# NUS-HPC-AI-Lab/Dynamic-Tuning

Hardware: AMD Instinct MI355X
Metric: images/sec DyT ViT-B/16 fine-tune step (student+teacher fwd, bwd, AdamW) @ keep~0.7 (higher is better)
Workload: dtype fp16; 1 GPU; ViT-B/16 DyT on CIFAR-100 shape, batch=128/GPU, 1xMI355X per rank, keep-ratio target 0.7 (BASELINE.json configs[1]; N>1 = configs[3] shape: global batch 128*N, DP over RCCL); per_gpu_batch=128, global_batch=128, ffn_num=64, num_classes=100, train_mode=compact, parallelism=dp1, hip_graph=False

## Files before the change

dynamic-tuning_amd/_lib.py:

```python
import ctypes
import os


_HERE = os.path.dirname(os.path.abspath(__file__))
_LIB_DIR = os.environ.get("DYT_LIB_DIR", _HERE)
LIB_PATH = os.path.join(_LIB_DIR, "libdyt_hip.so")
LIB_PATH_F16 = os.path.join(_LIB_DIR, "libdyt_hip_f16.so")

PREC_FP32, PREC_BF16 = 0, 1
PREC_FP16 = 2
PREC_FP16X3F = 4
PREC_FP16X3H = 5
PREC_FP16F8 = 6
PREC_FP16X3Q = 7
PREC_FP16X3 = 3
F_TRAINING, F_COMPLETE, F_SAVE, F_MASKED_DENSE, F_GATE_ALWAYS, F_ACCUM_GRAD, F_DEVICE_SEED, F_TOKENS_IN, F_TOKENS_OUT = 1, 2, 4, 8, 16, 32, 64, 128, 256
CREATE_WIDE_HEAD = 1
OPT_STREAM_OVERLAP, OPT_CLS_TAIL, OPT_SHARE_BLOCK0, OPT_COUNT_FLOPS_TOKENS, OPT_GRAD_SCALE_LOG2, OPT_FC2_CAT, OPT_ATTN_BWD_FUSED, OPT_F32_SPLIT16, OPT_ATTN_V2, OPT_GEMM_SPLITK, OPT_LEARNABLE_SCALE = 1, 2, 3, 4, 5, 6, 7, 8, 9, 10, 11

(P_CLS, P_POS, P_PE_W, P_PE_B, P_LN1_W, P_LN1_B, P_QKV_W, P_QKV_B, P_PROJ_W, P_PROJ_B, P_LN2_W, P_LN2_B,
 P_FC1_W, P_FC1_B, P_FC2_W, P_FC2_B, P_NORM_W, P_NORM_B, P_AD_DOWN_W, P_AD_DOWN_B, P_AD_UP_W, P_AD_UP_B,
 P_GATE_W, P_GATE_B, P_HEAD_W, P_HEAD_B,
 P_POOL_QUERY, P_POOL_NQ_W, P_POOL_NQ_B, P_POOL_NK_W, P_POOL_NK_B, P_POOL_NV_W, P_POOL_NV_B, P_POOL_Q_W, P_POOL_K_W,
 P_POOL_V_W, P_POOL_Q_BIAS, P_POOL_V_BIAS, P_POOL_PROJ_W, P_POOL_PROJ_B, P_AD_SCALE, P_AD_LN_W, P_AD_LN_B, P_COUNT) = range(44)
# ... 48 lines not shown
                ("inference_only", ctypes.c_int32)]


class DyTError(RuntimeError):
    pass


def inference_only_default(explicit=None, tuning_config=None):
    if explicit is not None:
        return bool(explicit)
    try:
        v = getattr(tuning_config, "dyt_inference_only")
    except (AttributeError, KeyError):
        v = None
    if v is not None:
        return bool(v)
    return os.environ.get("DYT_INFERENCE_ONLY", "0").strip().lower() not in ("", "0", "false", "no", "off")


def wide_head_default(explicit=None, tuning_config=None, num_classes=0):
    if explicit is not None:
        return bool(explicit)
    try:
        v = getattr(tuning_config, "dyt_wide_head")
    except (AttributeError, KeyError):
        v = None
    if v is not None:
        return bool(v)
    e = os.environ.get("DYT_WIDE_HEAD")
    if e is not None and e.strip() != "":
        return e.strip().lower() not in ("0", "false", "no", "off")
    return int(num_classes) > 1024


_lib = None

_vp, _i, _i64, _f, _u64 = ctypes.c_void_p, ctypes.c_int, ctypes.c_int64, ctypes.c_float, ctypes.c_uint64

SYMBOLS = {
    "dyt_last_error": (ctypes.c_char_p, []),
    "dyt_version": (_i, []),
    "dyt_operand_type": (_i, []),
    "dyt_ctx_create": (_i, [ctypes.POINTER(Config), ctypes.POINTER(_vp)]),
    "dyt_ctx_create_ex": (_i, [ctypes.POINTER(Config), ctypes.c_uint32, ctypes.POINTER(_vp)]),
    "dyt_ctx_destroy": (_i, [_vp]),
    "dyt_ctx_bytes": (_i, [_vp, ctypes.POINTER(_i64)]),
    "dyt_ctx_set_option": (_i, [_vp, _i, _i]),
    "dyt_set_global_option": (_i, [_i, _i]),
    "dyt_set_drop_path": (_i, [_vp, _f]),
    "dyt_set_drop_path_scales": (_i, [_vp, _i, _vp]),
    "dyt_set_soft_targets": (_i, [_vp, _vp, _i]),
    "dyt_set_frozen": (_i, [_vp, _i, _i, _vp, _vp]),
    "dyt_trainable_numel": (_i, [_vp, ctypes.POINTER(_i64)]),
    "dyt_trainable_offset": (_i, [_vp, _i, _i, ctypes.POINTER(_i64), ctypes.POINTER(_i64)]),
    "dyt_forward": (_i, [_vp, _i, _vp, _i, _i, _vp, _vp, _vp, _vp, _u64, _vp, _vp, _vp, _vp]),
    "dyt_backward": (_i, [_vp, _i, _vp, _vp, _vp, _vp, _vp, _vp]),
    "dyt_loss": (_i, [_vp, _i, _vp, _vp, _vp, _i, _f, _f, _f, _f, _vp, _vp, _vp, _vp, _vp]),
    "dyt_adamw": (_i, [_vp, _vp, _vp, _vp, _i64, _i, _f, _f, _f, _f, _f, _f, _vp]),
    "dyt_adamw_guarded": (_i, [_vp, _vp, _vp, _vp, _i64, _vp, _f, _f, _f, _f, _f, _f, _vp]),
    "dyt_step_fwd_bwd": (_i, [_vp, _vp, _vp, _i, _i, _vp, _vp, _vp, _vp, _u64, _f, _f, _f, _f, _vp, _vp, _vp, _vp,
                              _vp, _vp]),
    "dyt_seed": (_i, [_vp, _u64, _vp]),
    "dyt_grad_part": (_i, [_vp, _i, ctypes.POINTER(_i64), ctypes.POINTER(_i64)]),
    "dyt_stream_wait_grads": (_i, [_vp, _i, _vp]),
    "dyt_allreduce_grads": (_i, [_vp, _vp, _vp, _vp, _vp]),
    "dyt_clip_grad_norm": (_i, [_vp, _vp, _i64, _f, _f, _vp, _vp]),
    "dyt_debug_dispatch": (_i, [_vp, _i, _i, _vp, _vp, _vp, _vp, _vp]),
    "dyt_debug_dact": (_i, [_vp, _i, _i, _vp, _vp, _vp]),
    "dyt_debug_drop_path": (_i, [_vp, _i, _vp, _vp]),
    "dyt_layernorm": (_i, [_vp, _vp, _vp, _vp, _i, _vp]),
    "dyt_linear": (_i, [_vp, _vp, _vp, _vp, _i, _i, _i, _i, _vp]),
    "dyt_linear_split": (_i, [_vp, _vp, _vp, _vp, _i, _i, _i, _i, _vp]),
    "dyt_attention": (_i, [_vp, _vp, _vp, _vp, _i, _i, _vp]),
    "dyt_adapter_fwd": (_i, [_vp, _vp, _vp, _vp, _vp, _vp, _vp, _i, _i, _f, _f, _vp, _u64, _i, _vp]),
    "dyt_adapter_bwd": (_i, [_vp, _vp, _vp, _vp, _vp, _vp, _vp, _vp, _vp, _vp, _i, _i, _f, _f, _vp, _u64, _i, _vp]),
    "dyt_head_wide": (_i, [_vp, _vp, _vp, _vp, _vp, _vp, _vp, _vp, _vp, _vp, _i, _i, _vp]),
    "dyt_mlp_gathered_fwd": (_i, [_vp, _i, _vp, _vp, _vp, _i, _vp, _vp]),
    "dyt_mlp_gathered_bwd": (_i, [_vp, _i, _vp, _vp, _vp, _vp, _i, _vp]),
    "dyt_gate_compact": (_i, [_vp, _vp, _vp, _vp, _vp, _i, _i, _f, _f, _vp, _vp, _vp, _vp, _vp, _vp]),
    "dyt_gemm_bf16_raw": (_i, [_vp, _vp, _vp, _i, _i, _i, _i, _vp]),
    "dyt_gemm_f32_raw": (_i, [_vp, _vp, _vp, _i, _i, _i, _i, _vp]),
    "dyt_wgrad_scratch_floats": (ctypes.c_int64, [_i]),
    "dyt_wgrad_raw": (_i, [_vp, _vp, _i, _i, _i, _vp, _vp, _vp, _vp, _vp]),
    "dyt_debug_counters": (_i, [ctypes.POINTER(ctypes.c_uint64), _i]),
    "dyt_debug_checksums": (_i, [_i, ctypes.POINTER(ctypes.c_uint64), _i, ctypes.POINTER(_i)]),
    "dyt_debug_checksum_label": (ctypes.c_char_p, [_i, _i]),
    "dyt_debug_dump_read": (ctypes.c_int64, [_vp, _i64]),
    "dyt_profile_enable": (_i, [_vp, _i]),
    "dyt_profile_read": (_i, [_vp, _i, ctypes.POINTER(ctypes.c_double), ctypes.POINTER(_i64),
                              ctypes.POINTER(ctypes.c_double)]),
}


_lib16 = None


def lib(fp16=False):
    global _lib, _lib16
    if fp16:
        if _lib16 is None:
            lib()
            if not os.path.exists(LIB_PATH_F16):
                raise DyTError("%s not found: build it with `make -C dynamic-tuning_amd/csrc`" % LIB_PATH_F16)
            L = ctypes.CDLL(LIB_PATH_F16)
            for name, (res, args) in SYMBOLS.items():
                fn = getattr(L, name)
                fn.restype = res
                fn.argtypes = args
            if L.dyt_operand_type() != 1:
                raise DyTError("%s was not built with -DDYT_FP16" % LIB_PATH_F16)
            _lib16 = L
        return _lib16
    if _lib is None:
        if not os.path.exists(LIB_PATH):
            raise DyTError("%s not found: build it with `make -C dynamic-tuning_amd/csrc` "
                           "(or __graft_entry__.build()); the DyT path has no fallback" % LIB_PATH)
        import torch
        rt = os.path.join(os.path.dirname(torch.__file__), "lib", "libamdhip64.so")
        if not os.path.exists(rt):
            raise DyTError("PyTorch-ROCm's HIP runtime not found at %s" % rt)
        ctypes.CDLL(rt, mode=ctypes.RTLD_GLOBAL)
        rccl = os.path.join(os.path.dirname(torch.__file__), "lib", "librccl.so")
        if os.path.exists(rccl):
            ctypes.CDLL(rccl, mode=ctypes.RTLD_GLOBAL)
        L = ctypes.CDLL(LIB_PATH)
        for name, (res, args) in SYMBOLS.items():
            fn = getattr(L, name)
            fn.restype = res
            fn.argtypes = args
        _lib = L
    return _lib


def check(rc, L=None):
    if rc != 0:
        msg = (L or lib()).dyt_last_error().decode()
        if not msg and _lib16 is not None and L is None:
            msg = _lib16.dyt_last_error().decode()
        raise DyTError("libdyt_hip: %s (code %d)" % (msg, rc))


def ptr(t):
    if t is None:
        return None
    assert t.is_cuda and t.is_contiguous(), "libdyt_hip needs contiguous device tensors"
    return ctypes.c_void_p(t.data_ptr())


def stream_ptr():
    import torch
    return ctypes.c_void_p(torch.cuda.current_stream().cuda_stream)


class _NcclUniqueId(ctypes.Structure):
    _fields_ = [("internal", ctypes.c_byte * 128)]


_rccl = None


def rccl():
    global _rccl
    if _rccl is None:
        import torch
        path = os.path.join(os.path.dirname(torch.__file__), "lib", "librccl.so")
        if not os.path.exists(path):
# ... 62 lines not shown
```

dynamic-tuning_amd/csrc/rowops.hip:

```cpp
#include <stdlib.h>
#include <algorithm>
#include "kernels.h"
#include "rowhelp.h"

namespace dyt {

#define LAUNCH_CHECK() DYT_HIP_CHECK(hipGetLastError())

#if defined(DYT_NOPIN_LN) || defined(DYT_NOPIN_ROWS)
#define LN_ROWPIN(x)
#else
#define LN_ROWPIN(x) (x).landed()
#endif
#if defined(DYT_NOPIN_LN) || defined(DYT_NOPIN_SCALARS)
#define LN_SCALPIN3(a, b, c)
#else
#define LN_SCALPIN3(a, b, c) DYT_PIN3(a, b, c)
#endif
#if defined(DYT_NOPIN_TOK) || defined(DYT_NOPIN_ROWS)
#define TK_ROWPIN(x)
#else
#define TK_ROWPIN(x) (x).landed()
#endif
#if defined(DYT_NOPIN_TOK) || defined(DYT_NOPIN_SCALARS)
// ... 830 lines not shown
        for (int i = threadIdx.x; i < nparts; i += 64) acc += part[i];
        acc = wave_sum(acc);
        if (threadIdx.x == 0) {
            const float norm = sqrtf(acc) * fabsf(pre_scale);
            coef_s = fminf(1.0f, max_norm / (norm + 1e-6f));
            if (blockIdx.x == 0 && norm_out) norm_out[0] = norm;
        }
    }
    __syncthreads();
    const float coef = coef_s;
    if (coef >= 1.0f) return;
    for (int64_t i = (int64_t)blockIdx.x * 256 + threadIdx.x; i < n; i += (int64_t)gridDim.x * 256) g[i] *= coef;
}
int launch_clip_grad_norm(float* g, int64_t n, float max_norm, float pre_scale, float* scratch, float* norm_out, hipStream_t s) {
    const int nparts = 256;
    hipLaunchKernelGGL(sqsum_kernel, dim3(nparts), dim3(256), 0, s, g, n, scratch);
    hipLaunchKernelGGL(clip_scale_kernel, dim3(nparts), dim3(256), 0, s, g, n, scratch, nparts, max_norm, pre_scale, norm_out);
    LAUNCH_CHECK();
    return 0;
}

int launch_adamw(float* p, const float* g, float* m, float* v, int64_t n, float lr, float b1, float b2, float eps,
                 float wd, float bc1, float rsqrt_bc2, float gscale, hipStream_t s) {
    hipLaunchKernelGGL(adamw_kernel, dim3((unsigned)((n + 255) / 256)), dim3(256), 0, s, p, g, m, v, n, lr, b1, b2, eps,
                       wd, bc1, rsqrt_bc2, gscale);
    LAUNCH_CHECK();
    return 0;
}

template <class AT>
__global__ __launch_bounds__(256) void bwd_prep_kernel(const float* __restrict__ g, const AT* __restrict__ h,
                                                       const int* __restrict__ dst_of, const float* __restrict__ row_mask,
                                                       AT* __restrict__ g_at, AT* __restrict__ dH,
                                                       float* __restrict__ dmask, int M, float gs) {
    const int lane = threadIdx.x & 63;
    const int t = blockIdx.x * 4 + (threadIdx.x >> 6);
    if (t >= M) return;
    Row12 gr;
    gr.load(g + (size_t)t * D, lane);
    int r = dst_of ? dst_of[t] : t;
    float mk = row_mask ? row_mask[t] : 1.0f;
    gr.landed(); DYT_PIN2(r, mk);
    if (g_at) {
        Row12 gsc;
#pragma unroll
        for (int i = 0; i < 12; ++i) gsc.v[i] = gr.v[i] * gs;
        gsc.store(g_at + (size_t)t * D, lane);
    }
    float dm = 0.f;
    if (r >= 0) {
        if (h) {
            Row12 hr;
            hr.load_at(h + (size_t)r * D, lane);
            hr.landed();
            dm = dot12(gr, hr);
        }
        if (dH) {
            if (row_mask) {
#pragma unroll
                for (int i = 0; i < 12; ++i) gr.v[i] *= mk;
            }
#pragma unroll
            for (int i = 0; i < 12; ++i) gr.v[i] *= gs;
            gr.store(dH + (size_t)r * D, lane);
        }
    }
    if (dmask && lane == 0) dmask[t] = dm;
}
int launch_bwd_prep(int precision, const BwdPrepArgs& a, hipStream_t s) {
    const int grid = (a.M + 3) / 4;
    if (precision == 0)
        hipLaunchKernelGGL(bwd_prep_kernel<float>, dim3(grid), dim3(256), 0, s, a.g, (const float*)a.h, a.dst_of, a.row_mask,
                           (float*)a.g_at, (float*)a.dH, a.dmask, a.M, 1.0f);
    else
        hipLaunchKernelGGL(bwd_prep_kernel<bf16>, dim3(grid), dim3(256), 0, s, a.g, (const bf16*)a.h, a.dst_of, a.row_mask,
                           (bf16*)a.g_at, (bf16*)a.dH, a.dmask, a.M, a.gs);
    LAUNCH_CHECK();
    return 0;
}

constexpr int TOK_PER_BLOCK = 32;

template <class AT>
__global__ __launch_bounds__(256) void tok_bwd_kernel(TokBwdArgs a) {
    __shared__ float red[4][D + 1];
    const int tid = threadIdx.x, lane = tid & 63, wave = tid >> 6;
    Row12 wg, ln2w, dwg;
    float dbg = 0.f;
#pragma unroll
    for (int i = 0; i < 12; ++i) dwg.v[i] = 0.f;
    if (a.gate_w) { wg.load(a.gate_w, lane); TK_ROWPIN(wg); }
    if (a.dA2) { ln2w.load(a.ln2_w, lane); TK_ROWPIN(ln2w); }
    const int t0 = blockIdx.x * TOK_PER_BLOCK;
    int rv = -1;
    if (a.dA2 && a.write_du) {
        const int tt = t0 + wave + 4 * lane;
        if (lane < TOK_PER_BLOCK / 4 && tt < a.M) {
            if (a.g_cls) { const int bb = tt / NT; rv = (tt - bb * NT == 0) ? bb : -1; }
            else rv = a.dst_of ? a.dst_of[tt] : tt;
        }
    }
    for (int k = wave; k < TOK_PER_BLOCK; k += 4) {
        const int t = t0 + k;
        if (t >= a.M) break;
        const int b = t / NT, n = t - b * NT;
        Row12 du, ur, e, dy;
        const bool need_u = (a.dA2 && (!a.g_cls || n == 0)) || a.gate_w;
        const bool gate = a.gate_w && n >= 1;
        const bool cat = gate && a.cat_dact && a.dmask;
        if (need_u) ur.load_nt(a.u + (size_t)t * D, lane);
        const bool du16 = a.du_in_at && a.write_du && !a.g_cls;
        if (du16) du.load_at(reinterpret_cast<const AT*>(a.du_in_at) + (size_t)t * D, lane);
        else if (a.write_du && !a.g_cls) du.load(a.du + (size_t)t * D, lane);
        else if (a.write_du && n == 0) du.load(a.g_cls + (size_t)b * D, lane);
        else {
#pragma unroll
            for (int i = 0; i < 12; ++i) du.v[i] = 0.f;
        }
        if (a.dad) e.load_at(reinterpret_cast<const AT*>(a.dad) + (size_t)t * D, lane);
        const int r = __builtin_amdgcn_readlane(rv, k >> 2);
        if (r >= 0) dy.load_at(reinterpret_cast<const AT*>(a.dA2) + (size_t)r * D, lane);
        float2 st2 = make_float2(0.f, 1.f);
        if (a.dA2 && a.write_du) st2 = a.stats2[t];
        float ext = 0.f, sf = 0.f, dmk = 0.f, dlg = 0.f;
        float cd = 0.f, cz = 0.f;
        if (gate) {
            const size_t oi = (size_t)b * a.out_stride + n - 1;
            if (a.dtoken_select) ext = a.dtoken_select[oi];
            else if (a.dtok) ext = a.dtok[0] + (a.maskf[t] != 0.f ? a.dtok[2] : a.dtok[1]);
            sf = a.soft[t];
            if (a.dmask) dmk = a.dmask[t];
            if (a.dtoken_logits) dlg = a.dtoken_logits[oi];
            if (cat) {
                cd = to_f32(reinterpret_cast<const AT*>(a.cat_dact)[(size_t)t * RP + lane]);
                cz = to_f32(reinterpret_cast<const AT*>(a.cat_ddz)[(size_t)t * RP + lane]);
            }
        }
        if (need_u) TK_ROWPIN(ur);
        TK_ROWPIN(du);
        if (a.dad) TK_ROWPIN(e);
        if (r >= 0) TK_ROWPIN(dy);
        TK_SCALPIN3(st2.x, st2.y, ext);
        TK_SCALPIN3(sf, dmk, dlg);
        if (cat) {
            DYT_PIN2(cd, cz);
            const float czs = a.cat_ddz_dscale ? a.cat_ddz_scale * *a.cat_ddz_dscale : a.cat_ddz_scale;
            if (a.maskf[t] != 0.f) dmk -= wave_sum(cd * cz) * czs;
        }
        const float bs = a.branch_scale ? a.branch_scale[b] : 1.0f;
        dmk *= bs;
        if (du16) {
#pragma unroll
            for (int i = 0; i < 12; ++i) du.v[i] *= a.inv_gs;
        }
        if (a.dad) {
#pragma unroll
            for (int i = 0; i < 12; ++i) du.v[i] += e.v[i] * a.inv_gs;
        }
        if (a.dA2 && a.write_du) {
            if (r >= 0) {
                ln_bwd_row(dy, ur, ln2w, st2);
                const float ds = a.inv_gs * bs;
#pragma unroll
                for (int i = 0; i < 12; ++i) du.v[i] += dy.v[i] * ds;
            }
        }
        if (gate) {
            float dlogit = (dmk + ext) * sf * (1.0f - sf);
            if (a.training) dlogit /= a.tau;
            dlogit += dlg;
#pragma unroll
            for (int i = 0; i < 12; ++i) {
                du.v[i] = fmaf(dlogit, wg.v[i], du.v[i]);
                dwg.v[i] = fmaf(dlogit, ur.v[i], dwg.v[i]);
            }
            dbg += dlogit;
        }
        if (a.write_du) {
            if (a.du) du.store(a.du + (size_t)t * D, lane);
            if (a.du3) du.store_split3(reinterpret_cast<bf16*>(a.du3) + (size_t)t * SPLIT_A * D, lane, a.du3_scale, a.du3_hi_only);
            if (a.du_at) {
                Row12 dsc;
#pragma unroll
                for (int i = 0; i < 12; ++i) dsc.v[i] = du.v[i] * a.gs;
                dsc.store(reinterpret_cast<AT*>(a.du_at) + (size_t)t * D, lane);
            }
        }
    }
    if (a.gate_w) {
#pragma unroll
        for (int i = 0; i < 3; ++i)
#pragma unroll
            for (int e = 0; e < 4; ++e) red[wave][i * 256 + lane * 4 + e] = dwg.v[4 * i + e];
        if (lane == 0) red[wave][D] = dbg;
        __syncthreads();
        for (int c = tid; c < D + 1; c += 256)
            a.partial[(size_t)blockIdx.x * (D + 1) + c] = red[0][c] + red[1][c] + red[2][c] + red[3][c];
    }
}
int launch_tok_bwd(int precision, const TokBwdArgs& a, int* nblocks_out, hipStream_t s) {
    const int grid = (a.M + TOK_PER_BLOCK - 1) / TOK_PER_BLOCK;
    if (nblocks_out) *nblocks_out = grid;
    if (dbg_skip(8)) return 0;
    if (precision == 0) hipLaunchKernelGGL(tok_bwd_kernel<float>, dim3(grid), dim3(256), 0, s, a);
    else hipLaunchKernelGGL(tok_bwd_kernel<bf16>, dim3(grid), dim3(256), 0, s, a);
    LAUNCH_CHECK();
    return 0;
}

__global__ __launch_bounds__(256) void drop_path_draw_kernel(float* __restrict__ scales, int depth, int batch, float rate, uint64_t seed,
                                                             const uint64_t* __restrict__ seed_dev, uint64_t subseq_base) {
    const int i = blockIdx.x * 256 + threadIdx.x;
    if (i >= 2 * depth * batch) return;
    const int b = i % batch, l = (i / batch) % depth, branch = i / (batch * depth);
    const float drop = depth > 1 ? rate * (float)l / (float)(depth - 1) : 0.f;
    float v = 1.0f;
    if (drop > 0.f) {
        const float keep = 1.0f - drop;
        Philox ph(seed_dev ? *seed_dev : seed, subseq_base + (uint64_t)(2 * l + branch), (uint64_t)b);
        v = ph.u01(0) < keep ? 1.0f / keep : 0.0f;
    }
    scales[i] = v;
}
int launch_drop_path_draw(float* scales, int depth, int batch, float rate, uint64_t seed, const uint64_t* seed_dev, uint64_t subseq_base, hipStream_t s) {
    hipLaunchKernelGGL(drop_path_draw_kernel, dim3((2 * depth * batch + 255) / 256), dim3(256), 0, s, scales, depth, batch, rate, seed, seed_dev, subseq_base);
    LAUNCH_CHECK();
    return 0;
}
template <class AT>
__global__ __launch_bounds__(256) void scale_rows_kernel(AT* __restrict__ x, const float* __restrict__ scale, int M, int ld) {
    const size_t i = ((size_t)blockIdx.x * 256 + threadIdx.x) * 4;
    if (i >= (size_t)M * ld) return;
    const float sc = scale[(int)(i / ld) / NT];
    float v[4];
    load4(x + i, v);
    store4(x + i, v[0] * sc, v[1] * sc, v[2] * sc, v[3] * sc);
}
int launch_scale_rows(int precision, void* x, const float* scale, int M, int ld, hipStream_t s) {
    const unsigned grid = (unsigned)(((size_t)M * ld / 4 + 255) / 256);
    if (precision == 0) hipLaunchKernelGGL(scale_rows_kernel<float>, dim3(grid), dim3(256), 0, s, (float*)x, scale, M, ld);
    else hipLaunchKernelGGL(scale_rows_kernel<bf16>, dim3(grid), dim3(256), 0, s, (bf16*)x, scale, M, ld);
    LAUNCH_CHECK();
    return 0;
}

__global__ __launch_bounds__(256) void reduce_partials_kernel(const float* __restrict__ partial, int nparts, int stride,
                                                              float* __restrict__ out, int n, float alpha) {
    __shared__ float red[8][32];
    const int o = threadIdx.x & 31, grp = threadIdx.x >> 5;
    const int i = blockIdx.x * 32 + o;
    float acc = 0.f;
    if (i < n) {
        const int per = (nparts + 7) / 8;
        const int p0 = grp * per, p1 = min(nparts, p0 + per);
#pragma unroll 4
        for (int p = p0; p < p1; ++p) acc += partial[(size_t)p * stride + i];
    }
    red[grp][o] = acc;
    __syncthreads();
    if (grp == 0 && i < n) {
        float t = 0.f;
#pragma unroll
        for (int g = 0; g < 8; ++g) t += red[g][o];
        out[i] += alpha * t;
    }
}
int launch_reduce_partials(const float* partial, int nparts, int stride, float* out, int n, float alpha, hipStream_t s) {
    hipLaunchKernelGGL(reduce_partials_kernel, dim3((n + 31) / 32), dim3(256), 0, s, partial, nparts, stride, out, n, alpha);
    LAUNCH_CHECK();
    return 0;
}

struct TokReduceBatch { const float* partial[ReduceQueue::MAX_TOK]; float* out[ReduceQueue::MAX_TOK]; int nparts[ReduceQueue::MAX_TOK]; };
__global__ __launch_bounds__(256) void reduce_partials_batch_kernel(TokReduceBatch b, int stride, int n) {
    __shared__ float red[8][32];
    const float* __restrict__ partial = b.partial[blockIdx.y];
    const int nparts = b.nparts[blockIdx.y];
    const int o = threadIdx.x & 31, grp = threadIdx.x >> 5;
    const int i = blockIdx.x * 32 + o;
    float acc = 0.f;
    if (i < n) {
        const int per = (nparts + 7) / 8;
        const int p0 = grp * per, p1 = min(nparts, p0 + per);
#pragma unroll 4
        for (int p = p0; p < p1; ++p) acc += partial[(size_t)p * stride + i];
    }
    red[grp][o] = acc;
    __syncthreads();
// ... 333 lines not shown
```

dynamic-tuning_amd/csrc/unit_abi.hip:

```cpp
#include "ctx.h"

namespace dyt {

template <class AT>
__global__ void qkv_split_kernel(const float* __restrict__ qkv, AT* __restrict__ q, AT* __restrict__ k, AT* __restrict__ v,
                                 int batch) {
    const size_t idx = (size_t)blockIdx.x * 256 + threadIdx.x;
    if (idx >= (size_t)batch * NT * 3 * D) return;
    const int col = (int)(idx % (3 * D));
    const size_t row = idx / (3 * D);
    const int b = (int)(row / NT), n = (int)(row % NT);
    const int which = col / D, c = col % D, h = c >> 6, d = c & 63;
    const float val = qkv[idx] * (which == 0 ? 0.125f : 1.0f);
    AT* dst = which == 0 ? q : (which == 1 ? k : v);
    dst[(((size_t)b * NH + h) * NT + n) * HD + d] = from_f32<AT>(val);
}
template <class AT>
__global__ void to_f32_kernel(const AT* __restrict__ src, float* __restrict__ dst, size_t n) {
    const size_t i = (size_t)blockIdx.x * 256 + threadIdx.x;
    if (i < n) dst[i] = to_f32(src[i]);
}

}

extern "C" int dyt_debug_dact(dyt_ctx* c, int slot, int layer, float* out, int* rows_out, void* stream) {
    if (!c || !out || slot < 0 || slot >= c->cfg.slots || layer < 0 || layer >= c->cfg.depth) { set_error("bad slot / layer"); return DYT_ERR_ARG; }
    { int rc = refuse_inference(c, "dyt_debug_dact (per-block tensors of a saved pass)"); if (rc) return rc; }
    const Slot& S = c->slots[slot];
    if (S.batch < 1) { set_error("slot %d holds no pass", slot); return DYT_ERR_STATE; }
    hipStream_t s = static_cast<hipStream_t>(stream);
    const bool tail = c->cls_tail && layer == c->cfg.depth - 1;
    const size_t rows = tail ? (size_t)S.batch : (size_t)S.batch * NT, n = rows * RP;
    const LayerS& L = S.L[layer];
    if (rows_out) *rows_out = (int)rows;
    if (S.saved16 && L.dact16) hipLaunchKernelGGL(to_f32_kernel<bf16>, dim3((unsigned)((n + 255) / 256)), dim3(256), 0, s, (const bf16*)L.dact16, out, n);
    else if (c->prec == DYT_PREC_FP32) DYT_HIP_CHECK(hipMemcpyAsync(out, L.d_act, n * 4, hipMemcpyDeviceToDevice, s));
    else hipLaunchKernelGGL(to_f32_kernel<bf16>, dim3((unsigned)((n + 255) / 256)), dim3(256), 0, s, (const bf16*)L.d_act, out, n);
    DYT_HIP_CHECK(hipGetLastError());
    return DYT_OK;
}

extern "C" int dyt_gemm_bf16_raw(const void* a, const void* w, void* cmat, int M, int N, int K, int variant, void* stream) {
    if (!a || !w || !cmat) { set_error("null argument"); return DYT_ERR_ARG; }
    return launch_gemm_raw(a, w, cmat, M, N, K, variant, static_cast<hipStream_t>(stream));
}

extern "C" int64_t dyt_wgrad_scratch_floats(int M) { return (int64_t)((M + 511) / 512) * (D + 8) * 80; }
extern "C" int dyt_wgrad_raw(const void* X, const void* Y, int M, int r, int precision, float* partial, float* out_w, float* out_xsum,
                             float* out_ysum, void* stream) {
    if (!X || !Y || !partial || !out_w || M < 1 || r < 1 || r > RP) { set_error("bad argument"); return DYT_ERR_ARG; }
    WgradArgs a; a.X = X; a.Y = Y; a.M = M; a.r = r; a.partial = partial;
    a.out_w = out_w; a.sc = r; a.sj = 1; a.alpha = 1.0f; a.out_xsum = out_xsum; a.alpha_x = 1.0f; a.out_ysum = out_ysum; a.alpha_y = 1.0f;
    return launch_wgrad(precision, a, static_cast<hipStream_t>(stream));
}

extern "C" int dyt_gemm_f32_raw(const float* a, const float* w, float* cmat, int M, int N, int K, int variant, void* stream) {
    if (!a || !w || !cmat) { set_error("null argument"); return DYT_ERR_ARG; }
    return launch_gemm_f32_raw(a, w, cmat, M, N, K, variant, static_cast<hipStream_t>(stream));
}

extern "C" int dyt_debug_counters(uint64_t* out4, int reset) {
    if (!out4) { set_error("null argument"); return DYT_ERR_ARG; }
    return gemm_debug_counters(reinterpret_cast<unsigned long long*>(out4), reset);
}

extern "C" int dyt_layernorm(const float* x, const float* w, const float* b, float* out, int rows, void* stream) {
    if (!x || !w || !b || !out || rows < 1) { set_error("bad argument"); return DYT_ERR_ARG; }
    return launch_ln_fwd_f32out(x, w, b, out, rows, static_cast<hipStream_t>(stream));
}

struct Scratch {
    std::vector<void*> ptrs;
    ~Scratch() { for (void* p : ptrs) hipFree(p); }
    void* get(size_t bytes) {
        void* p = nullptr;
        if (hipMalloc(&p, bytes) != hipSuccess) return nullptr;
        ptrs.push_back(p);
        return p;
    }
};

extern "C" int dyt_linear(const float* a, const float* w, const float* bias, float* cmat, int M, int N, int K, int precision,
                          void* stream) {
    if (!a || !w || !cmat || M < 1) { set_error("bad argument"); return DYT_ERR_ARG; }
    hipStream_t s = static_cast<hipStream_t>(stream);
    GemmArgs g; g.M = M; g.N = N; g.K = K; g.bias = bias; g.out_f32 = cmat;
    Scratch sc;
    if (precision == 0) { g.A = a; g.W = w; }
    else {
        void* a2 = sc.get((size_t)M * K * 2); void* w2 = sc.get((size_t)N * K * 2);
        if (!a2 || !w2) { set_error("scratch alloc failed"); return DYT_ERR_HIP; }
        int rc = launch_convert(1, a, a2, (int64_t)M * K, s); if (rc) return rc;
        rc = launch_convert(1, w, w2, (int64_t)N * K, s); if (rc) return rc;
        g.A = a2; g.W = w2;
    }
    int rc = launch_gemm(precision, EPI_BIAS_F32, g, s);
    if (rc) return rc;
    DYT_HIP_CHECK(hipStreamSynchronize(s));
    return DYT_OK;
}

extern "C" int dyt_linear_split(const float* a, const float* w, const float* bias, float* cmat, int M, int N, int K, int form, void* stream) {
    if (!a || !w || !cmat || M < 1 || (form != 3 && form != 8)) { set_error("bad argument"); return DYT_ERR_ARG; }
    hipStream_t s = static_cast<hipStream_t>(stream);
    Scratch sc;
    void* a3 = sc.get((size_t)((M + 255) / 256 * 256) * SPLIT_A * K * 2); void* w3 = sc.get((size_t)N * SPLIT_A * K * 2);
    int* ew = (int*)sc.get(16); unsigned* scr = (unsigned*)sc.get(16);
    if (!a3 || !w3 || !ew || !scr) { set_error("scratch alloc failed"); return DYT_ERR_HIP; }
    int rc = form == 8 ? launch_split_w_f8(w, w3, N, K, ew, scr, s) : launch_split3_w(w, w3, N, K, s);
    if (rc) return rc;
    GemmArgs g; g.A = a; g.W = w; g.M = M; g.N = N; g.K = K; g.bias = bias; g.out_f32 = cmat; g.W3 = w3; g.a3 = a3;
    if (form == 8) { g.f8 = true; g.w_exp = ew; }
    rc = launch_gemm(0, EPI_BIAS_F32, g, s);
    if (rc) return rc;
    DYT_HIP_CHECK(hipStreamSynchronize(s));
    return DYT_OK;
}

template <class AT>
static int attention_test(const float* qkv, float* out, const float* dout, float* dqkv, int B, int P, hipStream_t s) {
    Scratch sc;
    const size_t M = (size_t)B * NT;
    AT* q = (AT*)sc.get(M * D * sizeof(AT)); AT* k = (AT*)sc.get(M * D * sizeof(AT)); AT* v = (AT*)sc.get(M * D * sizeof(AT));
    AT* o = (AT*)sc.get(M * D * sizeof(AT));
    float* lse = (float*)sc.get((size_t)B * NH * NT * 4);
    if (!q || !k || !v || !o || !lse) { set_error("scratch alloc failed"); return DYT_ERR_HIP; }
    const size_t n3 = M * 3 * D;
    hipLaunchKernelGGL(qkv_split_kernel<AT>, dim3((unsigned)((n3 + 255) / 256)), dim3(256), 0, s, qkv, q, k, v, B);
    int rc = launch_attn_fwd(P, q, k, v, o, lse, B, s);
    if (rc) return rc;
    hipLaunchKernelGGL(to_f32_kernel<AT>, dim3((unsigned)((M * D + 255) / 256)), dim3(256), 0, s, (const AT*)o, out, M * D);
    if (dout && dqkv) {
        AT* d_o = (AT*)sc.get(M * D * sizeof(AT)); AT* dq = (AT*)sc.get(n3 * sizeof(AT));
        float* delta = (float*)sc.get((size_t)B * NH * NT * 4);
        if (!d_o || !dq || !delta) { set_error("scratch alloc failed"); return DYT_ERR_HIP; }
        rc = launch_convert(P, dout, d_o, (int64_t)(M * D), s); if (rc) return rc;
// ... 302 lines not shown
```

include/dyt_hip.h:

```cpp
#ifndef DYT_HIP_H
#define DYT_HIP_H

#include <stdint.h>

#ifdef __cplusplus
extern "C" {
#endif

#define DYT_OK 0
#define DYT_ERR_ARG (-1)
#define DYT_ERR_HIP (-2)
#define DYT_ERR_STATE (-3)

#define DYT_PREC_FP32 0
#define DYT_PREC_BF16 1

#define DYT_F_TRAINING 1
#define DYT_F_COMPLETE 2
#define DYT_F_SAVE 4
#define DYT_F_MASKED_DENSE 8
#define DYT_F_ACCUM_GRAD 32
#define DYT_F_DEVICE_SEED 64
#define DYT_F_TOKENS_IN 128
#define DYT_F_TOKENS_OUT 256
// ... 70 lines not shown
int dyt_set_global_option(int option, int value);

int dyt_set_drop_path(dyt_ctx* ctx, float rate);
int dyt_set_drop_path_scales(dyt_ctx* ctx, int slot, const float* scales);

int dyt_set_frozen(dyt_ctx* ctx, int param, int layer, const float* src, void* stream);

int dyt_trainable_numel(const dyt_ctx* ctx, int64_t* numel);
int dyt_trainable_offset(const dyt_ctx* ctx, int param, int layer, int64_t* offset, int64_t* numel);

int dyt_forward(dyt_ctx* ctx, int slot, const float* images, int batch, int flags,
                const float* trainable, const float* g1, const float* g2,
                const uint8_t* keep_mask, uint64_t seed,
                float* logits, float* token_select, float* token_logits, void* stream);

int dyt_backward(dyt_ctx* ctx, int slot, const float* dlogits, const float* dtoken_select,
                 const float* dtok_uniform, const float* dtoken_logits, float* grad_flat, void* stream);

int dyt_loss(dyt_ctx* ctx, int slot_student, const float* logits_s, const float* logits_t,
             const int64_t* targets, int batch, float token_target_ratio, float token_loss_ratio,
             float token_minimal, float token_minimal_weight,
             float* dlogits_s, float* dlogits_t, float* out_losses, float* dtok, void* stream);

int dyt_set_soft_targets(dyt_ctx* ctx, const float* targets, int rows);

int dyt_adamw(float* param, const float* grad, float* exp_avg, float* exp_avg_sq, int64_t numel,
              int step, float lr, float beta1, float beta2, float eps, float weight_decay,
              float grad_scale, void* stream);

int dyt_adamw_guarded(float* param, const float* grad, float* exp_avg, float* exp_avg_sq, int64_t numel, int32_t* state,
                      float lr, float beta1, float beta2, float eps, float weight_decay, float grad_scale, void* stream);

int dyt_step_fwd_bwd(dyt_ctx* ctx, const float* images, const int64_t* targets, int batch,
                     int flags, const float* trainable,
                     const float* g1, const float* g2, const uint8_t* keep_mask, uint64_t seed,
                     float token_target_ratio, float token_loss_ratio,
                     float token_minimal, float token_minimal_weight,
                     float* grad_flat, float* out_losses, float* logits_s, float* logits_t,
                     float* token_select, void* stream);

int dyt_seed(dyt_ctx* ctx, uint64_t seed, void* stream);

int dyt_grad_part(const dyt_ctx* ctx, int part, int64_t* offset, int64_t* numel);
int dyt_stream_wait_grads(dyt_ctx* ctx, int part, void* stream);

int dyt_allreduce_grads(dyt_ctx* ctx, void* rccl_comm, float* grad_flat, void* comm_stream, void* stream);

int dyt_clip_grad_norm(dyt_ctx* ctx, float* grad, int64_t numel, float max_norm, float pre_scale, float* norm_out, void* stream);

int dyt_debug_dispatch(dyt_ctx* ctx, int slot, int layer, int32_t* row_src, int32_t* dst_of, int32_t* counts, int32_t* total,
                       void* stream);
int dyt_debug_dact(dyt_ctx* ctx, int slot, int layer, float* out, int* rows_out, void* stream);
int dyt_debug_drop_path(dyt_ctx* ctx, int slot, float* out, void* stream);

int dyt_adapter_fwd(const float* x, const float* down_w, const float* down_b, const float* up_w, const float* up_b,
                    const float* residual, float* out, int M, int r, float scale, float drop_p, const uint8_t* keep_mask,
                    uint64_t seed, int precision, void* stream);
int dyt_adapter_bwd(const float* x, const float* down_w, const float* down_b, const float* up_w, const float* dout, float* dx,
                    float* d_down_w, float* d_down_b, float* d_up_w, float* d_up_b, int M, int r, float scale, float drop_p,
                    const uint8_t* keep_mask, uint64_t seed, int precision, void* stream);
int dyt_head_wide(const float* cls_x, const float* norm_w, const float* norm_b, const float* head_w, const float* head_b,
                  float* logits, const float* dlogits, float* dx, float* d_head_w, float* d_head_b, int batch, int C, void* stream);
int dyt_mlp_gathered_fwd(dyt_ctx* ctx, int layer, const float* u, const float* mask, float* x, int batch, int32_t* total_out,
                         void* stream);
int dyt_mlp_gathered_bwd(dyt_ctx* ctx, int layer, const float* u, const float* mask, const float* dy, float* du, int batch, void* stream);

int dyt_linear_split(const float* a, const float* w, const float* bias, float* c, int M, int N, int K, int form, void* stream);

int dyt_layernorm(const float* x, const float* w, const float* b, float* out, int rows, void* stream);
int dyt_linear(const float* a, const float* w, const float* bias, float* c, int M, int N, int K,
               int precision, void* stream);
int dyt_attention(const float* qkv, float* out, const float* dout, float* dqkv, int batch,
                  int precision, void* stream);
int dyt_gate_compact(const float* u, const float* w, const float* b, const float* g1, const float* g2,
                     int batch, int training, float tau, float threshold,
                     float* mask, float* logits, int32_t* keep_idx, int32_t* counts, int32_t* total,
                     void* stream);

int dyt_gemm_bf16_raw(const void* a, const void* w, void* c, int M, int N, int K, int variant, void* stream);
int dyt_gemm_f32_raw(const float* a, const float* w, float* c, int M, int N, int K, int variant, void* stream);
int64_t dyt_wgrad_scratch_floats(int M);
int dyt_wgrad_raw(const void* X, const void* Y, int M, int r, int precision, float* partial, float* out_w, float* out_xsum,
                  float* out_ysum, void* stream);
int dyt_debug_checksums(int slot, uint64_t* out, int max_n, int* n_out);
const char* dyt_debug_checksum_label(int slot, int i);
int64_t dyt_debug_dump_read(void* dst_device, int64_t max_bytes);
int dyt_debug_counters(uint64_t* out4, int reset);
int dyt_profile_enable(dyt_ctx* ctx, int on);
int dyt_profile_read(dyt_ctx* ctx, int category, double* ms, int64_t* launches, double* flops);

#ifdef __cplusplus
}
#endif
#endif
```

Baseline: 5534 images/s.

## Specialize token-backward kernel by template and batch loads across tokens

Splits the token backward kernel into template variants keyed on gate, concat-dact and dA2 presence, so dead branches are removed at compile time. Gated variants load two tokens per wave before consuming either, to overlap memory latency. The ungated path gets a one-wave-per-token kernel. Loads half-precision rows packed rather than unpacked. Adds env-selectable schedules and a raw test entry point. The cost is more kernel instantiations and higher register pressure.

After: 5422 images/s. 2.0% lower.

```diff
diff --git a/dynamic-tuning_amd/_lib.py b/dynamic-tuning_amd/_lib.py
--- a/dynamic-tuning_amd/_lib.py
+++ b/dynamic-tuning_amd/_lib.py
@@ -154,6 +154,8 @@
     "dyt_gemm_f32_raw": (_i, [_vp, _vp, _vp, _i, _i, _i, _i, _vp]),
     "dyt_wgrad_scratch_floats": (ctypes.c_int64, [_i]),
     "dyt_wgrad_raw": (_i, [_vp, _vp, _i, _i, _i, _vp, _vp, _vp, _vp, _vp]),
+    "dyt_tok_bwd_raw": (_i, [_vp, _vp, _vp, _vp, _vp, _vp, _vp, _vp, _vp, _vp, _vp, _vp, _vp, _vp, _i, _i, _f, _vp, _vp, _i, _i, _f, _vp, _vp,
+                             _vp, _vp, _f, _vp, _vp, _vp, _f, _i, _i, ctypes.POINTER(_i), _vp]),
     "dyt_debug_counters": (_i, [ctypes.POINTER(ctypes.c_uint64), _i]),
     "dyt_debug_checksums": (_i, [_i, ctypes.POINTER(ctypes.c_uint64), _i, ctypes.POINTER(_i)]),
     "dyt_debug_checksum_label": (ctypes.c_char_p, [_i, _i]),
diff --git a/dynamic-tuning_amd/csrc/rowops.hip b/dynamic-tuning_amd/csrc/rowops.hip
--- a/dynamic-tuning_amd/csrc/rowops.hip
+++ b/dynamic-tuning_amd/csrc/rowops.hip
@@ -936,112 +936,188 @@
 constexpr int TOK_PER_BLOCK = 32;
 
 template <class AT>
-__global__ __launch_bounds__(256) void tok_bwd_kernel(TokBwdArgs a) {
-    __shared__ float red[4][D + 1];
+struct RowP {
+    typedef AT v4 __attribute__((ext_vector_type(4)));
+    v4 p[3];
+    __device__ __forceinline__ void load(const AT* q, int lane) {
+#pragma unroll
+        for (int i = 0; i < 3; ++i) p[i] = *reinterpret_cast<const v4*>(q + i * 256 + lane * 4);
+    }
+    __device__ __forceinline__ void landed() { DYT_PIN3(p[0], p[1], p[2]); }
+    __device__ __forceinline__ void unpack(Row12& o) const {
+#pragma unroll
+        for (int i = 0; i < 3; ++i)
+#pragma unroll
+            for (int e = 0; e < 4; ++e) o.v[4 * i + e] = to_f32(p[i][e]);
+    }
+};
+
+template <class AT>
+struct TokIn {
+    Row12 ur, du;
+    RowP<AT> e, dy;
+    float2 st2;
+    float ext, sf, dmk, dlg, cd, cz, mkf, bs;
+    int t, b, n, r;
+    bool need_u, gate, cat;
+};
+
+struct TokConst { float dt0, dt1, dt2, czs; };
+
+template <class AT, bool GATE, bool CAT, bool DA2>
+__device__ __forceinline__ void tok_issue(const TokBwdArgs& a, TokIn<AT>& q, int t, int r, int lane) {
+    const int b = t / NT, n = t - b * NT;
+    q.t = t; q.b = b; q.n = n; q.r = r;
+    q.need_u = (DA2 && (!a.g_cls || n == 0)) || GATE;
+    q.gate = GATE && n >= 1;
+    q.cat = CAT && q.gate;
+    if (q.need_u) q.ur.load_nt(a.u + (size_t)t * D, lane);
+    const bool du16 = a.du_in_at && a.write_du && !a.g_cls;
+    if (du16) q.du.load_at(reinterpret_cast<const AT*>(a.du_in_at) + (size_t)t * D, lane);
+    else if (a.write_du && !a.g_cls) q.du.load(a.du + (size_t)t * D, lane);
+    else if (a.write_du && n == 0) q.du.load(a.g_cls + (size_t)b * D, lane);
+    else {
+#pragma unroll
+        for (int i = 0; i < 12; ++i) q.du.v[i] = 0.f;
+    }
+    if (a.dad) q.e.load(reinterpret_cast<const AT*>(a.dad) + (size_t)t * D, lane);
+    if (r >= 0) q.dy.load(reinterpret_cast<const AT*>(a.dA2) + (size_t)r * D, lane);
+    q.st2 = make_float2(0.f, 1.f);
+    if (DA2 && a.write_du) q.st2 = a.stats2[t];
+    q.ext = 0.f; q.sf = 0.f; q.dmk = 0.f; q.dlg = 0.f; q.mkf = 0.f;
+    q.cd = 0.f; q.cz = 0.f;
+    if (q.gate) {
+        const size_t oi = (size_t)b * a.out_stride + n - 1;
+        if (a.dtoken_select) q.ext = a.dtoken_select[oi];
+        if ((CAT || (!a.dtoken_select && a.dtok)) && a.maskf) q.mkf = a.maskf[t];
+        q.sf = a.soft[t];
+        if (a.dmask) q.dmk = a.dmask[t];
+        if (a.dtoken_logits) q.dlg = a.dtoken_logits[oi];
+        if (CAT) {
+            q.cd = to_f32(reinterpret_cast<const AT*>(a.cat_dact)[(size_t)t * RP + lane]);
+            q.cz = to_f32(reinterpret_cast<const AT*>(a.cat_ddz)[(size_t)t * RP + lane]);
+        }
+    }
+    q.bs = a.branch_scale ? a.branch_scale[b] : 1.0f;
+}
+
+template <class AT, bool GATE, bool CAT>
+__device__ __forceinline__ void tok_drain(const TokBwdArgs& a, TokIn<AT>& q) {
+    if (q.need_u) TK_ROWPIN(q.ur);
+    TK_ROWPIN(q.du);
+    if (a.dad) TK_ROWPIN(q.e);
+    if (q.r >= 0) TK_ROWPIN(q.dy);
+    TK_SCALPIN3(q.st2.x, q.st2.y, q.bs);
+    if (GATE) {
+        TK_SCALPIN4(q.ext, q.sf, q.dmk, q.dlg);
+        TK_SCALPIN3(q.mkf, q.cd, q.cz);
+    }
+}
+
+template <class AT, bool GATE, bool CAT, bool DA2>
+__device__ __forceinline__ void tok_finish(const TokBwdArgs& a, TokIn<AT>& q, const TokConst& kc, const Row12& wg, const Row12& ln2w,
+                                           Row12& dwg, float& dbg, int lane) {
+    const int t = q.t;
+    float ext = q.ext, dmk = q.dmk;
+    if (q.gate && !a.dtoken_select && a.dtok) ext = kc.dt0 + (q.mkf != 0.f ? kc.dt2 : kc.dt1);
+    if (q.cat) {
+        if (q.mkf != 0.f) dmk -= wave_sum(q.cd * q.cz) * kc.czs;
+    }
+    const float bs = q.bs;
+    dmk *= bs;
+    Row12& du = q.du;
+    const bool du16 = a.du_in_at && a.write_du && !a.g_cls;
+    if (du16) {
+#pragma unroll
+        for (int i = 0; i < 12; ++i) du.v[i] *= a.inv_gs;
+    }
+    if (a.dad) {
+        Row12 e;
+        q.e.unpack(e);
+#pragma unroll
+        for (int i = 0; i < 12; ++i) du.v[i] += e.v[i] * a.inv_gs;
+    }
+    if (DA2 && a.write_du) {
+        if (q.r >= 0) {
+            Row12 dy;
+            q.dy.unpack(dy);
+            ln_bwd_row(dy, q.ur, ln2w, q.st2);
+            const float ds = a.inv_gs * bs;
+#pragma unroll
+            for (int i = 0; i < 12; ++i) du.v[i] += dy.v[i] * ds;
+        }
+    }
+    if (q.gate) {
+        float dlogit = (dmk + ext) * q.sf * (1.0f - q.sf);
+        if (a.training) dlogit /= a.tau;
+        dlogit += q.dlg;
+#pragma unroll
+        for (int i = 0; i < 12; ++i) {
+            du.v[i] = fmaf(dlogit, wg.v[i], du.v[i]);
+            dwg.v[i] = fmaf(dlogit, q.ur.v[i], dwg.v[i]);
+        }
+        dbg += dlogit;
+    }
+    if (a.write_du) {
+        if (a.du) du.store(a.du + (size_t)t * D, lane);
+        if (a.du3) du.store_split3(reinterpret_cast<bf16*>(a.du3) + (size_t)t * SPLIT_A * D, lane, a.du3_scale, a.du3_hi_only);
+        if (a.du_at) {
+            Row12 dsc;
+#pragma unroll
+            for (int i = 0; i < 12; ++i) dsc.v[i] = du.v[i] * a.gs;
+            dsc.store(reinterpret_cast<AT*>(a.du_at) + (size_t)t * D, lane);
+        }
+    }
+}
+
+template <bool GATE, bool CAT>
+__device__ __forceinline__ TokConst tok_consts(const TokBwdArgs& a) {
+    TokConst kc = {0.f, 0.f, 0.f, 0.f};
+    if (GATE && !a.dtoken_select && a.dtok) { kc.dt0 = a.dtok[0]; kc.dt1 = a.dtok[1]; kc.dt2 = a.dtok[2]; }
+    if (CAT) kc.czs = a.cat_ddz_dscale ? a.cat_ddz_scale * *a.cat_ddz_dscale : a.cat_ddz_scale;
+    return kc;
+}
+
+template <class AT, bool GATE, bool CAT, bool DA2, int NF, int WPE>
+__global__ __launch_bounds__(256, WPE) void tok_bwd_kernel(TokBwdArgs a) {
     const int tid = threadIdx.x, lane = tid & 63, wave = tid >> 6;
     Row12 wg, ln2w, dwg;
     float dbg = 0.f;
-#pragma unroll
-    for (int i = 0; i < 12; ++i) dwg.v[i] = 0.f;
-    if (a.gate_w) { wg.load(a.gate_w, lane); TK_ROWPIN(wg); }
-    if (a.dA2) { ln2w.load(a.ln2_w, lane); TK_ROWPIN(ln2w); }
+    if (GATE) {
+#pragma unroll
+        for (int i = 0; i < 12; ++i) dwg.v[i] = 0.f;
+        wg.load(a.gate_w, lane); TK_ROWPIN(wg);
+    }
+    if (DA2) { ln2w.load(a.ln2_w, lane); TK_ROWPIN(ln2w); }
+    const TokConst kc = tok_consts<GATE, CAT>(a);
     const int t0 = blockIdx.x * TOK_PER_BLOCK;
     int rv = -1;
-    if (a.dA2 && a.write_du) {
+    if (DA2 && a.write_du) {
         const int tt = t0 + wave + 4 * lane;
         if (lane < TOK_PER_BLOCK / 4 && tt < a.M) {
             if (a.g_cls) { const int bb = tt / NT; rv = (tt - bb * NT == 0) ? bb : -1; }
             else rv = a.dst_of ? a.dst_of[tt] : tt;
         }
     }
-    for (int k = wave; k < TOK_PER_BLOCK; k += 4) {
-        const int t = t0 + k;
-        if (t >= a.M) break;
-        const int b = t / NT, n = t - b * NT;
-        Row12 du, ur, e, dy;
-        const bool need_u = (a.dA2 && (!a.g_cls || n == 0)) || a.gate_w;
-        const bool gate = a.gate_w && n >= 1;
-        const bool cat = gate && a.cat_dact && a.dmask;
-        if (need_u) ur.load_nt(a.u + (size_t)t * D, lane);
-        const bool du16 = a.du_in_at && a.write_du && !a.g_cls;
-        if (du16) du.load_at(reinterpret_cast<const AT*>(a.du_in_at) + (size_t)t * D, lane);
-        else if (a.write_du && !a.g_cls) du.load(a.du + (size_t)t * D, lane);
-        else if (a.write_du && n == 0) du.load(a.g_cls + (size_t)b * D, lane);
-        else {
-#pragma unroll
-            for (int i = 0; i < 12; ++i) du.v[i] = 0.f;
-        }
-        if (a.dad) e.load_at(reinterpret_cast<const AT*>(a.dad) + (size_t)t * D, lane);
-        const int r = __builtin_amdgcn_readlane(rv, k >> 2);
-        if (r >= 0) dy.load_at(reinterpret_cast<const AT*>(a.dA2) + (size_t)r * D, lane);
-        float2 st2 = make_float2(0.f, 1.f);
-        if (a.dA2 && a.write_du) st2 = a.stats2[t];
-        float ext = 0.f, sf = 0.f, dmk = 0.f, dlg = 0.f;
-        float cd = 0.f, cz = 0.f;
-        if (gate) {
-            const size_t oi = (size_t)b * a.out_stride + n - 1;
-            if (a.dtoken_select) ext = a.dtoken_select[oi];
-            else if (a.dtok) ext = a.dtok[0] + (a.maskf[t] != 0.f ? a.dtok[2] : a.dtok[1]);
-            sf = a.soft[t];
-            if (a.dmask) dmk = a.dmask[t];
-            if (a.dtoken_logits) dlg = a.dtoken_logits[oi];
-            if (cat) {
-                cd = to_f32(reinterpret_cast<const AT*>(a.cat_dact)[(size_t)t * RP + lane]);
-                cz = to_f32(reinterpret_cast<const AT*>(a.cat_ddz)[(size_t)t * RP + lane]);
-            }
-        }
-        if (need_u) TK_ROWPIN(ur);
-        TK_ROWPIN(du);
-        if (a.dad) TK_ROWPIN(e);
-        if (r >= 0) TK_ROWPIN(dy);
-        TK_SCALPIN3(st2.x, st2.y, ext);
-        TK_SCALPIN3(sf, dmk, dlg);
-        if (cat) {
-            DYT_PIN2(cd, cz);
-            const float czs = a.cat_ddz_dscale ? a.cat_ddz_scale * *a.cat_ddz_dscale : a.cat_ddz_scale;
-            if (a.maskf[t] != 0.f) dmk -= wave_sum(cd * cz) * czs;
-        }
-        const float bs = a.branch_scale ? a.branch_scale[b] : 1.0f;
-        dmk *= bs;
-        if (du16) {
-#pragma unroll
-            for (int i = 0; i < 12; ++i) du.v[i] *= a.inv_gs;
-        }
-        if (a.dad) {
-#pragma unroll
-            for (int i = 0; i < 12; ++i) du.v[i] += e.v[i] * a.inv_gs;
-        }
-        if (a.dA2 && a.write_du) {
-            if (r >= 0) {
-                ln_bwd_row(dy, ur, ln2w, st2);
-                const float ds = a.inv_gs * bs;
-#pragma unroll
-                for (int i = 0; i < 12; ++i) du.v[i] += dy.v[i] * ds;
-            }
-        }
-        if (gate) {
-            float dlogit = (dmk + ext) * sf * (1.0f - sf);
-            if (a.training) dlogit /= a.tau;
-            dlogit += dlg;
-#pragma unroll
-            for (int i = 0; i < 12; ++i) {
-                du.v[i] = fmaf(dlogit, wg.v[i], du.v[i]);
-                dwg.v[i] = fmaf(dlogit, ur.v[i], dwg.v[i]);
-            }
-            dbg += dlogit;
-        }
-        if (a.write_du) {
-            if (a.du) du.store(a.du + (size_t)t * D, lane);
-            if (a.du3) du.store_split3(reinterpret_cast<bf16*>(a.du3) + (size_t)t * SPLIT_A * D, lane, a.du3_scale, a.du3_hi_only);
-            if (a.du_at) {
-                Row12 dsc;
-#pragma unroll
-                for (int i = 0; i < 12; ++i) dsc.v[i] = du.v[i] * a.gs;
-                dsc.store(reinterpret_cast<AT*>(a.du_at) + (size_t)t * D, lane);
-            }
-        }
-    }
-    if (a.gate_w) {
+    static_assert((TOK_PER_BLOCK / 4) % NF == 0, "a wave's tokens in groups of NF");
+    for (int k = wave; k < TOK_PER_BLOCK; k += 4 * NF) {
+        if (t0 + k >= a.M) break;
+        TokIn<AT> q[NF];
+#pragma unroll
+        for (int j = 0; j < NF; ++j) {
+            const int kk = k + 4 * j;
+            q[j].t = -1;
+            if (t0 + kk < a.M) tok_issue<AT, GATE, CAT, DA2>(a, q[j], t0 + kk, __builtin_amdgcn_readlane(rv, kk >> 2), lane);
+        }
+#pragma unroll
+        for (int j = 0; j < NF; ++j)
+            if (q[j].t >= 0) tok_drain<AT, GATE, CAT>(a, q[j]);
+#pragma unroll
+        for (int j = 0; j < NF; ++j)
+            if (q[j].t >= 0) tok_finish<AT, GATE, CAT, DA2>(a, q[j], kc, wg, ln2w, dwg, dbg, lane);
+    }
+    if constexpr (GATE) {
+        __shared__ float red[4][D + 1];
 #pragma unroll
         for (int i = 0; i < 3; ++i)
 #pragma unroll
@@ -1052,12 +1128,66 @@
             a.partial[(size_t)blockIdx.x * (D + 1) + c] = red[0][c] + red[1][c] + red[2][c] + red[3][c];
     }
 }
+
+template <class AT, bool DA2>
+__global__ __launch_bounds__(256) void tok_bwd_row_kernel(TokBwdArgs a) {
+    const int lane = threadIdx.x & 63;
+    const int t = blockIdx.x * 4 + (threadIdx.x >> 6);
+    if (t >= a.M) return;
+    Row12 ln2w, none;
+    float dbg = 0.f;
+    if (DA2) ln2w.load(a.ln2_w, lane);
+    int r = -1;
+    if (DA2 && a.write_du) {
+        if (a.g_cls) { const int bb = t / NT; r = (t - bb * NT == 0) ? bb : -1; }
+        else if (a.dst_of) { r = a.dst_of[t]; DYT_PIN1(r); }
+        else r = t;
+    }
+    const TokConst kc = {0.f, 0.f, 0.f, 0.f};
+    TokIn<AT> q;
+    tok_issue<AT, false, false, DA2>(a, q, t, r, lane);
+    if (DA2) TK_ROWPIN(ln2w);
+    tok_drain<AT, false, false>(a, q);
+    tok_finish<AT, false, false, DA2>(a, q, kc, none, ln2w, none, dbg, lane);
+}
+
+constexpr int TOK_NOGATE_DEFAULT = 1, TOK_GATE_DEFAULT = 2;
+
+template <class AT, bool GATE, bool CAT, bool DA2>
+static void tok_bwd_launch(const TokBwdArgs& a, int grid, int sched, hipStream_t s) {
+    if constexpr (!GATE) {
+        if (sched == 1) { hipLaunchKernelGGL((tok_bwd_row_kernel<AT, DA2>), dim3((a.M + 3) / 4), dim3(256), 0, s, a); return; }
+    }
+    if (sched == 3) hipLaunchKernelGGL((tok_bwd_kernel<AT, GATE, CAT, DA2, 2, 4>), dim3(grid), dim3(256), 0, s, a);
+    else if (sched == 2) hipLaunchKernelGGL((tok_bwd_kernel<AT, GATE, CAT, DA2, 2, 3>), dim3(grid), dim3(256), 0, s, a);
+    else if (sched == 1) hipLaunchKernelGGL((tok_bwd_kernel<AT, GATE, CAT, DA2, 1, 4>), dim3(grid), dim3(256), 0, s, a);
+    else hipLaunchKernelGGL((tok_bwd_kernel<AT, GATE, CAT, DA2, 1, 1>), dim3(grid), dim3(256), 0, s, a);
+}
+template <class AT>
+static void tok_bwd_pick(const TokBwdArgs& a, int grid, hipStream_t s) {
+    static const int nogate = getenv("DYT_TOK_BWD_NOGATE") ? atoi(getenv("DYT_TOK_BWD_NOGATE")) : TOK_NOGATE_DEFAULT;
+    static const int gate = getenv("DYT_TOK_BWD_GATE") ? atoi(getenv("DYT_TOK_BWD_GATE")) : TOK_GATE_DEFAULT;
+    const bool da2 = a.dA2 != nullptr;
+    if (!a.gate_w) {
+        if (da2) tok_bwd_launch<AT, false, false, true>(a, grid, nogate, s);
+        else tok_bwd_launch<AT, false, false, false>(a, grid, nogate, s);
+        return;
+    }
+    const bool cat = a.cat_dact && a.dmask;
+    if (cat) {
+        if (da2) tok_bwd_launch<AT, true, true, true>(a, grid, gate, s);
+        else tok_bwd_launch<AT, true, true, false>(a, grid, gate, s);
+    } else {
+        if (da2) tok_bwd_launch<AT, true, false, true>(a, grid, gate, s);
+        else tok_bwd_launch<AT, true, false, false>(a, grid, gate, s);
+    }
+}
 int launch_tok_bwd(int precision, const TokBwdArgs& a, int* nblocks_out, hipStream_t s) {
     const int grid = (a.M + TOK_PER_BLOCK - 1) / TOK_PER_BLOCK;
     if (nblocks_out) *nblocks_out = grid;
     if (dbg_skip(8)) return 0;
-    if (precision == 0) hipLaunchKernelGGL(tok_bwd_kernel<float>, dim3(grid), dim3(256), 0, s, a);
-    else hipLaunchKernelGGL(tok_bwd_kernel<bf16>, dim3(grid), dim3(256), 0, s, a);
+    if (precision == 0) tok_bwd_pick<float>(a, grid, s);
+    else tok_bwd_pick<bf16>(a, grid, s);
     LAUNCH_CHECK();
     return 0;
 }
diff --git a/dynamic-tuning_amd/csrc/unit_abi.hip b/dynamic-tuning_amd/csrc/unit_abi.hip
--- a/dynamic-tuning_amd/csrc/unit_abi.hip
+++ b/dynamic-tuning_amd/csrc/unit_abi.hip
@@ -52,6 +52,32 @@
     WgradArgs a; a.X = X; a.Y = Y; a.M = M; a.r = r; a.partial = partial;
     a.out_w = out_w; a.sc = r; a.sj = 1; a.alpha = 1.0f; a.out_xsum = out_xsum; a.alpha_x = 1.0f; a.out_ysum = out_ysum; a.alpha_y = 1.0f;
     return launch_wgrad(precision, a, static_cast<hipStream_t>(stream));
+}
+
+extern "C" int dyt_tok_bwd_raw(float* du, const void* du_in_at, const void* dA2, const int32_t* dst_of, const float* u, const float* stats2,
+                               const float* ln2_w, const float* gate_w, const float* soft, const float* maskf, const float* dmask,
+                               const float* dtoken_select, const float* dtoken_logits, const float* dtok, int out_stride, int training,
+                               float tau, void* du_at, float* partial, int M, int write_du, float gs, const void* dad, const float* g_cls,
+                               const void* cat_dact, const void* cat_ddz, float cat_ddz_scale, const float* cat_ddz_dscale,
+                               const float* branch_scale, void* du3, float du3_scale, int du3_hi_only, int precision, int* nblocks_out,
+                               void* stream) {
+    if (!u || M < 1 || !(gs > 0.f) || (precision != 0 && precision != 1)) { set_error("dyt_tok_bwd_raw: bad argument"); return DYT_ERR_ARG; }
+    if (dA2 && (!stats2 || !ln2_w)) { set_error("dyt_tok_bwd_raw: dA2 needs stats2 and ln2_w"); return DYT_ERR_ARG; }
+    if (gate_w && (!soft || !maskf || !partial || !(tau > 0.f))) { set_error("dyt_tok_bwd_raw: the gate needs soft, maskf, partial and tau > 0"); return DYT_ERR_ARG; }
+    if (write_du && !g_cls && !du && !du_in_at) { set_error("dyt_tok_bwd_raw: write_du needs du, du_in_at or g_cls"); return DYT_ERR_ARG; }
+    if ((cat_dact != nullptr) != (cat_ddz != nullptr)) { set_error("dyt_tok_bwd_raw: cat_dact and cat_ddz go together"); return DYT_ERR_ARG; }
+    TokBwdArgs a;
+    a.du = du; a.du_in_at = du_in_at; a.dA2 = dA2; a.dst_of = dst_of; a.u = u; a.stats2 = reinterpret_cast<const float2*>(stats2); a.ln2_w = ln2_w;
+    a.gate_w = gate_w; a.soft = soft; a.maskf = maskf; a.dmask = dmask; a.dtoken_select = dtoken_select; a.dtoken_logits = dtoken_logits;
+    a.dtok = dtok; a.out_stride = out_stride; a.training = training; a.tau = tau; a.du_at = du_at; a.partial = partial; a.M = M;
+    a.write_du = write_du; a.gs = gs; a.inv_gs = 1.0f / gs; a.dad = dad; a.g_cls = g_cls;
+    a.cat_dact = cat_dact; a.cat_ddz = cat_ddz; a.cat_ddz_scale = cat_ddz_scale; a.cat_ddz_dscale = cat_ddz_dscale;
+    a.branch_scale = branch_scale; a.du3 = du3; a.du3_scale = du3_scale; a.du3_hi_only = du3_hi_only != 0;
+    hipStream_t s = static_cast<hipStream_t>(stream);
+    int rc = launch_tok_bwd(precision, a, nblocks_out, s);
+    if (rc) return rc;
+    DYT_HIP_CHECK(hipStreamSynchronize(s));
+    return DYT_OK;
 }
 
 extern "C" int dyt_gemm_f32_raw(const float* a, const float* w, float* cmat, int M, int N, int K, int variant, void* stream) {
diff --git a/include/dyt_hip.h b/include/dyt_hip.h
--- a/include/dyt_hip.h
+++ b/include/dyt_hip.h
@@ -176,6 +176,13 @@
 int64_t dyt_wgrad_scratch_floats(int M);
 int dyt_wgrad_raw(const void* X, const void* Y, int M, int r, int precision, float* partial, float* out_w, float* out_xsum,
                   float* out_ysum, void* stream);
+int dyt_tok_bwd_raw(float* du, const void* du_in_at, const void* dA2, const int32_t* dst_of, const float* u, const float* stats2,
+                    const float* ln2_w, const float* gate_w, const float* soft, const float* maskf, const float* dmask,
+                    const float* dtoken_select, const float* dtoken_logits, const float* dtok, int out_stride, int training,
+                    float tau, void* du_at, float* partial, int M, int write_du, float gs, const void* dad, const float* g_cls,
+                    const void* cat_dact, const void* cat_ddz, float cat_ddz_scale, const float* cat_ddz_dscale,
+                    const float* branch_scale, void* du3, float du3_scale, int du3_hi_only, int precision, int* nblocks_out,
+                    void* stream);
 int dyt_debug_checksums(int slot, uint64_t* out, int max_n, int* n_out);
 const char* dyt_debug_checksum_label(int slot, int i);
 int64_t dyt_debug_dump_read(void* dst_device, int64_t max_bytes);
```
